# Victarry/Image-Generation-models

Measured on AMD Instinct MI355X. Metric: ddpm_cifar10_32x32_train_images_per_sec, higher is better.
Workload: dtype bf16; 1 GPU; DDPM CIFAR-10 32x32, UNet 128/1-2-4, T=1000 (BASELINE configs[1]): train step B=128/GPU + hipGraph denoise step B=64; per_gpu_batch=128, global_batch=128, parallelism=dp1, step_launch=hipGraph replay, denoise_batch=64, rccl_ranks=1, state_finite=True, matmul=bf16 MFMA, fp32 accumulate

## Files before the change

### image-generation-models_amd/csrc/small_channel.hip

```cpp
#include <stdlib.h>
#include "common.h"

namespace {

typedef float f32x4 __attribute__((ext_vector_type(4)));

template <bool B16> __device__ __forceinline__ f32x4 ldq(const void* base, size_t off) {
    if constexpr (B16) {
        const uint2 u = *reinterpret_cast<const uint2*>(reinterpret_cast<const uint16_t*>(base) + off);
        return f32x4{__uint_as_float(u.x << 16), __uint_as_float(u.x & 0xffff0000u), __uint_as_float(u.y << 16), __uint_as_float(u.y & 0xffff0000u)};
    } else return *reinterpret_cast<const f32x4*>(reinterpret_cast<const float*>(base) + off);
}
template <bool B16> __device__ __forceinline__ void stq(void* base, size_t off, const f32x4& v) {
    if constexpr (B16) *reinterpret_cast<uint2*>(reinterpret_cast<uint16_t*>(base) + off) = make_uint2(pack_bf16(v.x, v.y), pack_bf16(v.z, v.w));
    else *reinterpret_cast<f32x4*>(reinterpret_cast<float*>(base) + off) = v;
}

constexpr int WG_BLOCKS = 768;

template <bool POW2>
__device__ __forceinline__ void decode_px(int m, int H, int W, int w_sh, int hw_sh, int& n, int& yy, int& xx) {
    if constexpr (POW2) {
        n = m >> hw_sh; const int rem = m & ((1 << hw_sh) - 1);
        yy = rem >> w_sh; xx = rem & ((1 << w_sh) - 1);
    } else {
        n = m / (H * W); const int rem = m - n * (H * W);
        yy = rem / W; xx = rem - yy * W;
    }
}

template <int CIN, bool VEC>
__device__ __forceinline__ f32x4 load_small(const float* __restrict__ x, int ldx, int n, int iy, int ix, int H, int W) {
    const bool ok = iy >= 0 && iy < H && ix >= 0 && ix < W;
    const float* p = x + (size_t)((n * H + (ok ? iy : 0)) * W + (ok ? ix : 0)) * ldx;
    f32x4 v = {0.f, 0.f, 0.f, 0.f};
    if constexpr (VEC) v = *reinterpret_cast<const f32x4*>(p);
    else { v.x = p[0]; if (CIN > 1) v.y = p[1]; if (CIN > 2) v.z = p[2]; if (CIN > 3) v.w = p[3]; }
    const float k = ok ? 1.f : 0.f;
    return v * k;
}

template <int CIN, int KS, bool POW2, bool VEC>
__global__ __launch_bounds__(256) void small_cin_fwd_kernel(int N, int H, int W, int Cout, const float* __restrict__ x, int ldx,
                                                            const float* __restrict__ w, const float* __restrict__ bias,
                                                            float* __restrict__ y, int ldy, int w_sh, int hw_sh) {
    constexpr int NT = KS * KS;
    const int nq = Cout / 4;
    const int q = threadIdx.x % nq, psub = threadIdx.x / nq, pp = 256 / nq;
    f32x4 wr[NT * CIN];
#pragma unroll
    for (int i = 0; i < NT * CIN; ++i) wr[i] = *reinterpret_cast<const f32x4*>(w + (size_t)i * Cout + 4 * q);
// ... 112 lines not shown
#pragma unroll
            for (int k = 0; k < 3; ++k) a[i] += *reinterpret_cast<const f32x4*>(&red[((k * NA + i) * nq + l) * 4]);
    }
}

template <int CIN, int KS, bool POW2, bool VEC>
__global__ __launch_bounds__(256) void small_cin_wgrad_kernel(int N, int H, int W, int Cout, const float* __restrict__ x, int ldx,
                                                              const float* __restrict__ dy, int lddy, float* __restrict__ dW,
                                                              float* __restrict__ ws, int w_sh, int hw_sh) {
    constexpr int NT = KS * KS, NA = NT * CIN;
    extern __shared__ float red[];
    const int nq = Cout / 4;
    const int q = threadIdx.x % nq, psub = threadIdx.x / nq, pp = 256 / nq;
    f32x4 acc[NA];
#pragma unroll
    for (int i = 0; i < NA; ++i) acc[i] = f32x4{0.f, 0.f, 0.f, 0.f};
    const int M = N * H * W;
    const int per = (M + gridDim.x - 1) / gridDim.x;
    const int mb = blockIdx.x * per, me = min(M, mb + per);
    int m = mb + psub;
    f32x4 g = *reinterpret_cast<const f32x4*>(dy + (size_t)min(m, M - 1) * lddy + 4 * q);
    for (; m < me; m += pp) {
        const f32x4 gnext = *reinterpret_cast<const f32x4*>(dy + (size_t)min(m + pp, M - 1) * lddy + 4 * q);
        int n, yy, xx;
        decode_px<POW2>(m, H, W, w_sh, hw_sh, n, yy, xx);
#pragma unroll
        for (int tp = 0; tp < NT; ++tp) {
            const f32x4 xv = load_small<CIN, VEC>(x, ldx, n, yy + tp / KS - KS / 2, xx + tp % KS - KS / 2, H, W);
#pragma unroll
            for (int ci = 0; ci < CIN; ++ci) acc[tp * CIN + ci] += xv[ci] * g;
        }
        g = gnext;
    }
    block_reduce_quads<NA>(acc, nq, red);
    if (threadIdx.x < nq) {
        if (ws) {
            float* out = ws + (size_t)blockIdx.x * NA * Cout;
#pragma unroll
            for (int i = 0; i < NA; ++i) *reinterpret_cast<f32x4*>(out + (size_t)i * Cout + 4 * q) = acc[i];
        } else {
#pragma unroll
            for (int i = 0; i < NA; ++i)
#pragma unroll
                for (int k = 0; k < 4; ++k) atomicAdd(dW + (size_t)i * Cout + 4 * q + k, acc[i][k]);
        }
    }
}

template <int CIN, bool DY16 = false>
__global__ __launch_bounds__(256) void small_cin3x3_wgrad_tiled_kernel(int N, int H, int W, int Cout, const float* __restrict__ x, int ldx,
                                                                       const void* __restrict__ dy, int lddy, float* __restrict__ dW,
                                                                       float* __restrict__ ws, int w_sh, int ntiles) {
    constexpr int NA = 9 * CIN;
    extern __shared__ __attribute__((aligned(16))) float smem[];
    const int nq = Cout / 4;
    const int q = threadIdx.x % nq, psub = threadIdx.x / nq, pp = 256 / nq;
    const int rows = 64 >> w_sh, W2 = W + 2, HP = (rows + 2) * W2, tiles_per_img = H / rows;
    float* red = smem;
    float* halo_s = smem + (size_t)3 * NA * nq * 4;
    f32x4 acc[NA];
#pragma unroll
    for (int i = 0; i < NA; ++i) acc[i] = f32x4{0.f, 0.f, 0.f, 0.f};
    const int hp = threadIdx.x, hy = hp / W2, hx = hp - hy * W2;
    auto fetch = [&](int tile) -> f32x4 {
        const int n = tile / tiles_per_img, y0 = (tile - n * tiles_per_img) * rows;
        const int iy = y0 + hy - 1, ix = hx - 1;
// ... 22 lines not shown
#pragma unroll
            for (int k = 0; k < MAXPX; ++k) {
                const int px = base + k * pp;
                if (px < 64) {
                    const int ty = px >> w_sh, tx = px & (W - 1);
#pragma unroll
                    for (int tp = 0; tp < 9; ++tp) {
                        const f32x4 xv = *reinterpret_cast<const f32x4*>(hs + (size_t)((ty + tp / 3) * W2 + tx + tp % 3) * 4);
#pragma unroll
                        for (int ci = 0; ci < CIN; ++ci) acc[tp * CIN + ci] += xv[ci] * g[k];
                    }
                }
            }
        }
        buf ^= 1;
        if (hp < HP) *reinterpret_cast<f32x4*>(halo_s + ((size_t)buf * HP + hp) * 4) = nxt;
        __syncthreads();
    }
    block_reduce_quads<NA>(acc, nq, red);
    if (threadIdx.x < nq) {
        if (ws) {
            float* out = ws + (size_t)blockIdx.x * NA * Cout;
#pragma unroll
            for (int i = 0; i < NA; ++i) *reinterpret_cast<f32x4*>(out + (size_t)i * Cout + 4 * q) = acc[i];
        } else {
#pragma unroll
            for (int i = 0; i < NA; ++i)
#pragma unroll
                for (int k = 0; k < 4; ++k) atomicAdd(dW + (size_t)i * Cout + 4 * q + k, acc[i][k]);
        }
    }
}

__global__ __launch_bounds__(256) void partial_sum_kernel(const float* __restrict__ ws, int nparts, int nout, float* __restrict__ out, int rows4) {
    __shared__ float red[8][32];
    const int ol = threadIdx.x & 31, grp = threadIdx.x >> 5;
    const int o = blockIdx.x * 32 + ol;
    float s = 0.f;
    if (o < nout) {
        float s0 = 0.f, s1 = 0.f, s2 = 0.f, s3 = 0.f;
        int p = grp;
        for (; p + 56 < nparts; p += 64) {
            float v[8];
#pragma unroll
            for (int u = 0; u < 8; ++u) v[u] = ws[(size_t)(p + 8 * u) * nout + o];
            s0 += v[0] + v[4]; s1 += v[1] + v[5]; s2 += v[2] + v[6]; s3 += v[3] + v[7];
        }
        for (; p < nparts; p += 8) s0 += ws[(size_t)p * nout + o];
        s = (s0 + s1) + (s2 + s3);
    }
    red[grp][ol] = s;
    __syncthreads();
    if (grp == 0 && o < nout) {
#pragma unroll
        for (int g = 1; g < 8; ++g) s += red[g][ol];
        if (rows4 > 0) { if ((o & 3) < rows4) out[(o >> 2) * rows4 + (o & 3)] += s; }
        else out[o] += s;
    }
}

template <int CK, bool X16 = false>
__global__ __launch_bounds__(256) void small_cout_fwd_kernel(int M, int Cs, const void* __restrict__ x, int ldx,
                                                             const float* __restrict__ w, const float* __restrict__ bias,
                                                             float* __restrict__ y, int ldy) {
    const int sub = threadIdx.x & 7, pl = threadIdx.x >> 3;
    f32x4 wr[CK][4];
// ... 167 lines not shown
    const int mb = blockIdx.x * per, me = min(M, mb + per);
    int m = mb + psub;
    f32x4 xv = ldq<X16>(x, (size_t)min(m, M - 1) * ldx + 4 * q);
    for (; m < me; m += pp) {
        const f32x4 xnext = ldq<X16>(x, (size_t)min(m + pp, M - 1) * ldx + 4 * q);
        const float* gp = dy + (size_t)m * lddy;
        const f32x4 g = {gp[0], Cs > 1 ? gp[1] : 0.f, Cs > 2 ? gp[2] : 0.f, Cs > 3 ? gp[3] : 0.f};
#pragma unroll
        for (int e = 0; e < 4; ++e) acc[e] += xv[e] * g;
        if constexpr (DG) {
            f32x4 o;
#pragma unroll
            for (int e = 0; e < 4; ++e) { const f32x4 pr = g * wr[e]; o[e] = (pr.x + pr.y) + (pr.z + pr.w); }
            const size_t po = (size_t)m * lddx + 4 * q;
            if (dacc) o += ldq<DX16>(dx, po);
            stq<DX16>(dx, po, o);
        }
        xv = xnext;
    }
    block_reduce_quads<4>(acc, nq, red);
    if (threadIdx.x < nq) {
        if (ws) {
            float* out = ws + (size_t)blockIdx.x * C * 4;
#pragma unroll
            for (int e = 0; e < 4; ++e) *reinterpret_cast<f32x4*>(out + (size_t)(4 * q + e) * 4) = acc[e];
        } else {
#pragma unroll
            for (int e = 0; e < 4; ++e)
                for (int j = 0; j < Cs; ++j) atomicAdd(dW + (size_t)(4 * q + e) * Cs + j, acc[e][j]);
        }
    }
}

int log2_exact(int v) { int s = 0; while ((1 << s) < v) ++s; return (1 << s) == v ? s : -1; }

}

extern "C" size_t mi_conv_small_wgrad_workspace(int outputs) { return (size_t)WG_BLOCKS * (size_t)outputs * sizeof(float); }

namespace {
bool cin_tiled_geom(int ks, int H, int W, int ldx, const void* x) {
    const int w_sh = log2_exact(W), hw_sh = log2_exact(H * W);
    const int rows = w_sh >= 0 && W <= 64 ? 64 / W : 0;
    return ks == 3 && w_sh >= 0 && hw_sh >= 0 && ldx == 4 && ((uintptr_t)x & 15) == 0 && rows >= 1 && H % rows == 0 && (rows + 2) * (W + 2) <= 256;
}
}

extern "C" int mi_conv_small_cin_bf16_supported(int ks, int N, int H, int W, int Cin, int Cout, int ldx) {
    static const int tiled = (int)mi_knob("MI_SMALL_CIN_TILED", 1);
    return (tiled && N > 0 && Cin >= 1 && Cin <= 4 && (Cout == 64 || Cout == 128 || Cout == 256) && ((long)N * H * W) % 64 == 0 && cin_tiled_geom(ks, H, W, ldx, nullptr) &&
            (size_t)3 * 9 * Cin * (Cout / 4) * 16 <= 48 * 1024) ? 1 : 0;
}

extern "C" int mi_conv_small_cin_fwd_io(int ks, int N, int H, int W, int Cin, int Cout, const float* x, int ldx, const float* w,
                                        const float* bias, void* yv, int ldy, int y_bf16, void* stream) {
    MI_REQUIRE(x && w && yv && (ks == 1 || ks == 3) && Cin >= 1 && Cin <= 4 && Cout >= 4 && Cout % 4 == 0 && Cout <= 1024 && 256 % (Cout / 4) == 0 &&
               ldy % 4 == 0 && (((uintptr_t)yv & (y_bf16 ? 7 : 15)) | ((uintptr_t)w & 15)) == 0,
               "needs ks 1|3, Cin <= 4, Cout a multiple of 4 with Cout/4 dividing 256, 16-byte aligned y / w");
    float* y = (float*)yv;
    const int pp = 256 / (Cout / 4);
    long blocks = ((long)N * H * W + 2 * pp - 1) / (2 * pp); if (blocks > 4096) blocks = 4096;
    const int w_sh = log2_exact(W), hw_sh = log2_exact(H * W);
    const bool pow2 = w_sh >= 0 && hw_sh >= 0;
    const bool vec = ldx % 4 == 0 && ((uintptr_t)x & 15) == 0;
    hipStream_t st = (hipStream_t)stream;
    {
        static const int tiled = (int)mi_knob("MI_SMALL_CIN_TILED", 1);
        const int rows = w_sh >= 0 && W <= 64 ? 64 / W : 0;
// ... 55 lines not shown
    hipStream_t st = (hipStream_t)stream;
#define MI_TILED2(CIN) do { \
        if (y3_bf16) hipLaunchKernelGGL((small_cin3x3_fwd_tiled_kernel<CIN, true, true>), dim3(grid), dim3(256), lds, st, N, H, W, Cout, x, ldx, w3, bias3, y3, ldy3, w_sh, ntiles, w1, bias1, y1, ldy1, (unsigned long long*)ch.zero, (int)(ch.zero_bytes / 8), ch.gsrc, ch.gidx, ch.gdst, ch.grow, ch.gB); \
        else hipLaunchKernelGGL((small_cin3x3_fwd_tiled_kernel<CIN, false, true>), dim3(grid), dim3(256), lds, st, N, H, W, Cout, x, ldx, w3, bias3, y3, ldy3, w_sh, ntiles, w1, bias1, y1, ldy1, (unsigned long long*)ch.zero, (int)(ch.zero_bytes / 8), ch.gsrc, ch.gidx, ch.gdst, ch.grow, ch.gB); } while (0)
    switch (Cin) { case 1: MI_TILED2(1); break; case 2: MI_TILED2(2); break; case 3: MI_TILED2(3); break; default: MI_TILED2(4); break; }
#undef MI_TILED2
    MI_LAUNCH_CHECK();
    return 0;
}
extern "C" int mi_conv_small_cin_fwd(int ks, int N, int H, int W, int Cin, int Cout, const float* x, int ldx, const float* w,
                                     const float* bias, float* y, int ldy, void* stream) {
    return mi_conv_small_cin_fwd_io(ks, N, H, W, Cin, Cout, x, ldx, w, bias, y, ldy, 0, stream);
}

extern "C" int mi_conv_small_cin_wgrad_io(int ks, int N, int H, int W, int Cin, int Cout, const float* x, int ldx, const void* dyv,
                                          int lddy, int dy_bf16, float* dW, void* workspace, size_t ws_bytes, void* stream) {
    const int na = ks * ks * Cin;
    MI_REQUIRE(x && dyv && dW && (ks == 1 || ks == 3) && Cin >= 1 && Cin <= 4 && (Cout == 64 || Cout == 128 || Cout == 256) && lddy % 4 == 0 &&
               ((uintptr_t)dyv & (dy_bf16 ? 7 : 15)) == 0 && (size_t)3 * na * (Cout / 4) * 16 <= 48 * 1024,
               "needs ks 1|3, Cin <= 4, Cout in {64, 128, 256} with 3 ks ks Cin (Cout / 4) float4 of reduce area <= 48 KiB (3x3: Cin Cout <= 455), 16-byte aligned dy rows");
    const float* dy = (const float*)dyv;
    float* ws = (workspace && ws_bytes >= mi_conv_small_wgrad_workspace(na * Cout)) ? (float*)workspace : nullptr;
    const int w_sh = log2_exact(W), hw_sh = log2_exact(H * W);
    const bool pow2 = w_sh >= 0 && hw_sh >= 0;
    const bool vec = ldx % 4 == 0 && ((uintptr_t)x & 15) == 0;
    const size_t lds = (size_t)3 * na * (Cout / 4) * 4 * sizeof(float);
    hipStream_t st = (hipStream_t)stream;
    {
        static const int tiled = (int)mi_knob("MI_SMALL_CIN_TILED", 1);
        const int rows = w_sh >= 0 && W <= 64 ? 64 / W : 0;
        if (tiled && cin_tiled_geom(ks, H, W, ldx, x) && (Cout >= 128 || dy_bf16) && ((long)N * H * W) % 64 == 0) {
            const int ntiles = N * H * W / 64;
            const size_t lds2 = lds + (size_t)2 * (rows + 2) * (W + 2) * 16;
#define MI_TILED(CIN) do { \
                if (dy_bf16) hipLaunchKernelGGL((small_cin3x3_wgrad_tiled_kernel<CIN, true>), dim3(WG_BLOCKS), dim3(256), lds2, st, N, H, W, Cout, x, ldx, dyv, lddy, dW, ws, w_sh, ntiles); \
                else hipLaunchKernelGGL((small_cin3x3_wgrad_tiled_kernel<CIN, false>), dim3(WG_BLOCKS), dim3(256), lds2, st, N, H, W, Cout, x, ldx, dyv, lddy, dW, ws, w_sh, ntiles); } while (0)
            switch (Cin) { case 1: MI_TILED(1); break; case 2: MI_TILED(2); break; case 3: MI_TILED(3); break; default: MI_TILED(4); break; }
#undef MI_TILED
            if (ws) hipLaunchKernelGGL(partial_sum_kernel, dim3((na * Cout + 31) / 32), dim3(256), 0, st, ws, WG_BLOCKS, na * Cout, dW, 0);
            MI_LAUNCH_CHECK();
            return 0;
        }
    }
    MI_REQUIRE(!dy_bf16, "bf16 dy: only on the whole-row-tile kernel (mi_conv_small_cin_bf16_supported)");
#define MI_GO(CIN, KS) do { \
        if (pow2 && vec) hipLaunchKernelGGL((small_cin_wgrad_kernel<CIN, KS, true, true>), dim3(WG_BLOCKS), dim3(256), lds, st, N, H, W, Cout, x, ldx, dy, lddy, dW, ws, w_sh, hw_sh); \
        else if (vec) hipLaunchKernelGGL((small_cin_wgrad_kernel<CIN, KS, false, true>), dim3(WG_BLOCKS), dim3(256), lds, st, N, H, W, Cout, x, ldx, dy, lddy, dW, ws, 0, 0); \
        else hipLaunchKernelGGL((small_cin_wgrad_kernel<CIN, KS, false, false>), dim3(WG_BLOCKS), dim3(256), lds, st, N, H, W, Cout, x, ldx, dy, lddy, dW, ws, 0, 0); } while (0)
    if (ks == 3) MI_GO_CIN(3); else MI_GO_CIN(1);
#undef MI_GO
#undef MI_GO_CIN
    if (ws) hipLaunchKernelGGL(partial_sum_kernel, dim3((na * Cout + 31) / 32), dim3(256), 0, st, ws, WG_BLOCKS, na * Cout, dW, 0);
    MI_LAUNCH_CHECK();
    return 0;
}
extern "C" int mi_conv_small_cin_wgrad(int ks, int N, int H, int W, int Cin, int Cout, const float* x, int ldx, const float* dy,
                                       int lddy, float* dW, void* workspace, size_t ws_bytes, void* stream) {
    return mi_conv_small_cin_wgrad_io(ks, N, H, W, Cin, Cout, x, ldx, dy, lddy, 0, dW, workspace, ws_bytes, stream);
}

extern "C" int mi_conv3x3_small_cin_fwd(int N, int H, int W, int Cin, int Cout, const float* x, int ldx, const float* w,
                                        const float* bias, float* y, int ldy, void* stream) {
    return mi_conv_small_cin_fwd(3, N, H, W, Cin, Cout, x, ldx, w, bias, y, ldy, stream);
}
extern "C" int mi_conv3x3_small_cin_wgrad(int N, int H, int W, int Cin, int Cout, const float* x, int ldx, const float* dy,
                                          int lddy, float* dW, void* stream) {
    return mi_conv_small_cin_wgrad(3, N, H, W, Cin, Cout, x, ldx, dy, lddy, dW, nullptr, 0, stream);
}

extern "C" int mi_conv1x1_small_cout_io(int op, int M, int C, int Cs, const void* a, int lda, const float* b, int ldb,
                                        const float* w, const float* bias, void* out, int ldo, int accumulate, int wide_bf16,
                                        void* workspace, size_t ws_bytes, void* stream) {
    MI_REQUIRE(a && out && (op == 2 || w) && Cs >= 1 && Cs <= 4 && (C == 32 || C == 64 || C == 128 || C == 256) && M > 0,
               "needs Cs <= 4 and C in {32, 64, 128, 256}");
    hipStream_t st = (hipStream_t)stream;
    const uintptr_t wal = wide_bf16 ? 7 : 15;
    if (op == 0) {
        MI_REQUIRE(C <= 128 && lda % 4 == 0 && ((uintptr_t)a & wal) == 0, "forward: C <= 128, 16-byte (bf16: 8-byte) aligned x rows");
        int blocks = (M + 31) / 32; if (blocks > 1024) blocks = 1024;
#define MI_FWD(CK) do { \
            if (wide_bf16) hipLaunchKernelGGL((small_cout_fwd_kernel<CK, true>), dim3(blocks), dim3(256), 0, st, M, Cs, a, lda, w, bias, (float*)out, ldo); \
            else hipLaunchKernelGGL((small_cout_fwd_kernel<CK, false>), dim3(blocks), dim3(256), 0, st, M, Cs, a, lda, w, bias, (float*)out, ldo); } while (0)
        if (C == 128) MI_FWD(4); else if (C == 64) MI_FWD(2); else MI_FWD(1);
#undef MI_FWD
    } else if (op == 1) {
        MI_REQUIRE(ldo % 4 == 0 && ((uintptr_t)out & wal) == 0, "dgrad: 16-byte (bf16: 8-byte) aligned dx rows");
        const int pp = 256 / (C / 4);
        long blocks = ((long)M + pp - 1) / pp; if (blocks > 4096) blocks = 4096;
        if (wide_bf16) hipLaunchKernelGGL(small_cout_dgrad_kernel<true>, dim3((unsigned)blocks), dim3(256), 0, st, M, C, Cs, (const float*)a, lda, w, out, ldo, accumulate);
        else hipLaunchKernelGGL(small_cout_dgrad_kernel<false>, dim3((unsigned)blocks), dim3(256), 0, st, M, C, Cs, (const float*)a, lda, w, out, ldo, accumulate);
    } else if (op == 2) {
        MI_REQUIRE(b && C >= 64 && lda % 4 == 0 && ((uintptr_t)a & wal) == 0, "wgrad: needs dy, C in {64, 128, 256}, aligned x rows");
        float* ws = (workspace && ws_bytes >= mi_conv_small_wgrad_workspace(C * 4)) ? (float*)workspace : nullptr;
        const size_t lds = (size_t)3 * 4 * (C / 4) * 4 * sizeof(float);
        if (wide_bf16) hipLaunchKernelGGL(small_cout_wgrad_kernel<true>, dim3(WG_BLOCKS), dim3(256), lds, st, M, C, Cs, a, lda, b, ldb, (float*)out, ws);
        else hipLaunchKernelGGL(small_cout_wgrad_kernel<false>, dim3(WG_BLOCKS), dim3(256), lds, st, M, C, Cs, a, lda, b, ldb, (float*)out, ws);
        if (ws) hipLaunchKernelGGL(partial_sum_kernel, dim3((C * 4 + 31) / 32), dim3(256), 0, st, ws, WG_BLOCKS, C * 4, (float*)out, Cs);
    } else {
        return mi_set_error(-1, "mi_conv1x1_small_cout: op must be 0, 1 or 2");
    }
    MI_LAUNCH_CHECK();
    return 0;
}

extern "C" int mi_conv1x1_small_cout_gn_supported(int C, int Cs, int G) {
    return ((C == 64 || C == 128) && Cs >= 1 && Cs <= 4 && G > 0 && C % G == 0 && (C / G) % 16 == 0) ? 1 : 0;
}
extern "C" int mi_conv1x1_small_cout_gn_fwd(int M, int HW, int C, int Cs, const void* x_bf16, int ldx, const void* sums, const float* gamma,
                                            const float* beta, int G, float eps, const float* w, const float* bias, float* y, int ldy, void* stream) {
    MI_REQUIRE(x_bf16 && sums && gamma && beta && w && y && M > 0 && HW > 0 && M % HW == 0 && mi_conv1x1_small_cout_gn_supported(C, Cs, G) &&
               ldx % 4 == 0 && ldy == 4 && (((uintptr_t)x_bf16 & 7) | ((uintptr_t)sums & 15) | ((uintptr_t)gamma & 15) | ((uintptr_t)beta & 15) | ((uintptr_t)y & 15)) == 0,
               "needs C in {64, 128}, (C / G) % 16 == 0, Cs <= 4, y as padded 4-channel pixels, aligned operands");
    int ppw = 32;
    while ((long)M / ppw > 768 && HW % (2 * ppw) == 0) ppw *= 2;
    const int blocks = (M + ppw - 1) / ppw;
    hipStream_t st = (hipStream_t)stream;
    if (C == 128) hipLaunchKernelGGL((small_cout_fwd_gn_kernel<4>), dim3(blocks), dim3(256), 0, st, M, HW, Cs, (const uint16_t*)x_bf16, ldx, (const long long*)sums, gamma, beta, G, eps, w, bias, y, ldy, ppw);
    else hipLaunchKernelGGL((small_cout_fwd_gn_kernel<2>), dim3(blocks), dim3(256), 0, st, M, HW, Cs, (const uint16_t*)x_bf16, ldx, (const long long*)sums, gamma, beta, G, eps, w, bias, y, ldy, ppw);
    MI_LAUNCH_CHECK();
    return 0;
}

extern "C" int mi_conv1x1_small_cout_bwd(int M, int C, int Cs, const void* x, int ldx, int x_bf16, const float* dy, int lddy, const float* w,
                                         float* dW, void* dx, int lddx, int dx_bf16, int accumulate_dx, void* workspace, size_t ws_bytes, void* stream) {
    MI_REQUIRE(x && dy && w && dW && dx && Cs >= 1 && Cs <= 4 && (C == 64 || C == 128 || C == 256) && M > 0 && ldx % 4 == 0 && lddx % 4 == 0 &&
               ((uintptr_t)x & (x_bf16 ? 7 : 15)) == 0 && ((uintptr_t)dx & (dx_bf16 ? 7 : 15)) == 0, "needs Cs <= 4, C in {64, 128, 256}, aligned rows");
    hipStream_t st = (hipStream_t)stream;
    float* ws = (workspace && ws_bytes >= mi_conv_small_wgrad_workspace(C * 4)) ? (float*)workspace : nullptr;
    const size_t lds = (size_t)3 * 4 * (C / 4) * 4 * sizeof(float);
#define MI_BWD(X16, D16) hipLaunchKernelGGL((small_cout_wgrad_kernel<X16, true, D16>), dim3(WG_BLOCKS), dim3(256), lds, st, M, C, Cs, x, ldx, dy, lddy, dW, ws, w, dx, lddx, accumulate_dx)
    if (x_bf16) { if (dx_bf16) MI_BWD(true, true); else MI_BWD(true, false); }
    else { if (dx_bf16) MI_BWD(false, true); else MI_BWD(false, false); }
#undef MI_BWD
    if (ws) hipLaunchKernelGGL(partial_sum_kernel, dim3((C * 4 + 31) / 32), dim3(256), 0, st, ws, WG_BLOCKS, C * 4, dW, Cs);
    MI_LAUNCH_CHECK();
    return 0;
}

extern "C" int mi_conv1x1_small_cout_ws(int op, int M, int C, int Cs, const float* a, int lda, const float* b, int ldb,
                                        const float* w, const float* bias, float* out, int ldo, int accumulate,
                                        void* workspace, size_t ws_bytes, void* stream) {
    return mi_conv1x1_small_cout_io(op, M, C, Cs, a, lda, b, ldb, w, bias, out, ldo, accumulate, 0, workspace, ws_bytes, stream);
}

extern "C" int mi_conv1x1_small_cout(int op, int M, int C, int Cs, const float* a, int lda, const float* b, int ldb,
                                     const float* w, const float* bias, float* out, int ldo, int accumulate, void* stream) {
    return mi_conv1x1_small_cout_ws(op, M, C, Cs, a, lda, b, ldb, w, bias, out, ldo, accumulate, nullptr, 0, stream);
}
```

### image-generation-models_amd/src/ops/lib.py

```python
from __future__ import annotations

import ctypes as C
import os

_PKG_ROOT = os.path.dirname(os.path.dirname(os.path.dirname(os.path.abspath(__file__))))
_LIB = None


def library_path() -> str:
    return os.environ.get("MI_DDPM_LIB", os.path.join(_PKG_ROOT, "lib", "libmi_ddpm.so"))


class MiConvDesc(C.Structure):
    _fields_ = [(n, C.c_int) for n in (
        "N", "IH", "IW", "OH", "OW", "K", "Nc", "KH", "KW", "stride", "pad", "transposed", "w_kn", "mode",
        "K1", "ldx", "ldx2", "ldy", "ldr", "accumulate")]


class MiWgradDesc(C.Structure):
    _fields_ = [(n, C.c_int) for n in (
        "N", "GH", "GW", "DH", "DW", "Ci", "Cj", "KH", "KW", "stride", "pad", "gather_i", "mode", "I1",
        "ldp", "ldp2", "ldq")]


# ... 143 lines not shown
    "mi_conv_small_cin_bf16_supported": [_I, _I, _I, _I, _I, _I, _I],
    "mi_conv_small_cin_fwd": [_I, _I, _I, _I, _I, _I, _P, _I, _P, _P, _P, _I, _P],
    "mi_conv_small_cin_wgrad": [_I, _I, _I, _I, _I, _I, _P, _I, _P, _I, _P, _P, _Z, _P],
    "mi_conv_wgrad": [C.POINTER(MiWgradDesc), _P, _P, _P, _P, _P],
    "mi_conv3x3_wgrad": [C.POINTER(MiWgradDesc), _P, _P, _P, _P, _P],
    "mi_conv3x3_wgrad_supported": [C.POINTER(MiWgradDesc)],
    "mi_conv3x3_wgrad_ws": [C.POINTER(MiWgradDesc), _P, _P, _P, _P, _P, _Z, _P],
    "mi_conv3x3_wgrad_bias": [C.POINTER(MiWgradDesc), _P, _P, _P, _P, _P, _P, _Z, _P],
    "mi_colsum": [_I, _I, _P, _I, _P, _P],
    "mi_colsum_ordered": [_I, _I, _P, _I, _P, _P, _Z, _P],
    "mi_conv_wgrad_slabs": [C.POINTER(MiWgradDesc), _P, _P, _P, _P, _P, _Z, _P],
    "mi_gn_mish_fwd": [C.POINTER(MiGnDesc), _P, _P, _P, _P, _I, _P, _P, _P, _P],
    "mi_gn_mish_bwd": [C.POINTER(MiGnDesc), _P, _P, _P, _P, _P, _I, _P, _I, _P, _P, _P, _I, _P, _P],
    "mi_chan_layernorm_fwd": [_I, _I, _P, _I, _P, _P, _F, _P, _I, _P],
    "mi_chan_layernorm_bwd": [_I, _I, _P, _I, _P, _F, _P, _I, _P, _I, _I, _P, _P, _P],
    "mi_linattn_fwd": [_I, _I, _I, _P, _P, _P, _P, _P],
    "mi_linattn_bwd": [_I, _I, _I, _P, _P, _P, _P, _P, _P],
    "mi_vq_partials": [_I],
    "mi_vq_nearest_fwd": [_I, _I, _I, _P, _I, _P, _P, _P, _I, _P, _P],
    "mi_vq_bwd": [_I, _I, _I, _P, _I, _P, _P, _F, _F, _P, _P, _I, _I, _P, _P],
    "mi_vq_scatter_rows": [_I, _I, _I, _P, _I, _P, _P, _P],
    "mi_small_gemm": [_I, _I, _I, _I, _I, _P, _I, _P, _I, _P, _P, _I, _I, _I, _P],
    "mi_small_gemm_supported": [_I, _I, _I, _I, _I, _I, _I],
    "mi_linattn_fwd_io": [_I, _I, _I, _P, _P, _P, _P, _I, _P],
    "mi_linattn_bwd_io": [_I, _I, _I, _P, _P, _P, _P, _P, _I, _P],
    "mi_linattn_fwd_ws": [_I, _I, _I, _P, _P, _P, _P, _I, _P, _Z, _P],
    "mi_linattn_bwd_ws": [_I, _I, _I, _P, _P, _P, _P, _P, _I, _P, _Z, _P],
    "mi_chan_layernorm_fwd_io": [_I, _I, _P, _I, _P, _P, _F, _P, _I, _I, _P],
    "mi_chan_layernorm_bwd_io": [_I, _I, _P, _I, _P, _F, _P, _I, _P, _I, _I, _P, _P, _I, _P],
    "mi_chan_layernorm_bwd_part": [_I, _I, _P, _I, _P, _F, _P, _I, _P, _I, _I, _P, _I, _P],
    "mi_chan_layernorm_bwd_out": [_I, _I, _P, _I, _P, _F, _P, _I, _P, _I, _P, _I, _P, _P, _P, _I, _P],
    "mi_chan_layernorm_bwd_pipelined": [_I, _P, _P, _P, _P, _I, _I, _I, _I, _I],
    "mi_debug_ln_bwd_pipeline": [_I],
    "mi_rowsum_batch": [_I, _P, _P],
    "mi_f32_to_bf16_colsum_part": [_Z, _I, _P, _I, _P, _I, _P, _Z, C.POINTER(C.c_int), _P],
    "mi_time_embed": [_I, _I, _P, _P, _P],
    "mi_sample_norm_supported": [_I, _I, _I],
    "mi_sample_norm_fwd": [_I, _I, _I, _P, _P, _P, _P, _P, _F, _P],
    "mi_sample_norm_bwd": [_I, _I, _I, _P, _P, _P, _P, _P, _P, _P, _P, _P],
    "mi_sample_norm_bwd2": [_I, _I, _I, _P, _P, _P, _P, _P, _P, _P, _P, _P],
    "mi_leaky_relu_fwd": [_Z, _P, _P, _F, _P],
    "mi_leaky_relu_bwd": [_Z, _P, _P, _P, _F, _P],
    "mi_tanh_fwd": [_Z, _P, _P, _P],
    "mi_tanh_bwd": [_Z, _P, _P, _P, _P],
    "mi_lerp_rows": [_I, _Z, _P, _P, _P, _P, _P],
    "mi_gp_penalty": [_I, _Z, _P, _P, _P, _F, _P, _P],
    "mi_batchnorm_workspace": [_I],
    "mi_batchnorm_fwd": [_I, _I, _P, _P, _P, _P, _P, _P, _P, _P, _F, _F, _I, _P, _P],
    "mi_batchnorm_bwd": [_I, _I, _P, _P, _P, _P, _P, _P, _P, _P, _P, _P],
    "mi_vae_latent_fwd": [_I, _I, _P, _I, _P, _P, _P, _P],
    "mi_vae_latent_bwd": [_I, _I, _P, _I, _P, _P, _F, _P, _P, _I, _P],
    "mi_cvae_pack_input": [_I, _I, _I, _I, _P, _P, _P, _I, _P],
    "mi_cvae_latent_fwd": [_I, _I, _I, _P, _I, _P, _P, _P, _P, _P, _P],
    "mi_cvae_latent_bwd": [_I, _I, _I, _P, _I, _P, _P, _P, _I, _F, _P, _P, _P, _P],
    "mi_latent_disc_supported": [_I, _I, _I],
    "mi_latent_disc_fwd": [_I, _I, _I, _P, _I, _P, _I, _P, _P, _P, _I, _F, _F, _P, _P, _P, _P, _P, _P],
    "mi_latent_disc_bwd": [_I, _I, _I, _P, _I, _P, _I, _P, _P, _P, _I, _F, _P, _P, _P, _F, _I, _P, _I, _F, _I, _P],
    "mi_latent_disc_ln_supported": [_I, _I, _I, _I],
    "mi_latent_disc_ln_fwd": [_I, _I, _I, _I, _P, _I, _P, _I, _P, _I, _F, _F, _P, _P, _P],
    "mi_latent_disc_ln_bwd": [_I, _I, _I, _I, _P, _I, _P, _I, _P, _I, _F, _F, _F, _F, _P, _P, _P, _F, _I, _P, _I, _F, _I, _P],
    "mi_bn_seg_rows_per_workgroup": [_I, _I],
    "mi_bn_seg_fwd": [_I, _I, _I, _P, _P, _P, _P, _P, _P, _P, _P, _F, _F, _I, _I, _F, _P, _P],
    "mi_bn_seg_bwd": [_I, _I, _I, _P, _P, _P, _P, _P, _P, _P, _P, _P, _I, _I, _F, _P, _P],
    "mi_adv_loss": [_I, _I, _I, C.POINTER(C.c_int), _F, _P, _I, _P, _P, _P, _I, _P],
    "mi_info_latent": [_I, _I, _I, _I, _I, _P, _P, _I, _P, _I, _P, _I, _P],
    "mi_info_head_supported": [_I, _I, _I, _I, _I, _I, _I],
# ... 121 lines not shown
```

### include/mi_ddpm.h

```cpp
#ifndef MI_DDPM_H
#define MI_DDPM_H
#include <stddef.h>
#include <stdint.h>

#ifdef __cplusplus
extern "C" {
#endif

#define MI_ABI_VERSION 4
#define MI_MODE_FP32 0
#define MI_MODE_BF16 1

int mi_abi_version(void);
const char* mi_last_error(void);

typedef struct MiConvDesc {
    int N;
    int IH, IW;
    int OH, OW;
    int K;
    int Nc;
    int KH, KW, stride, pad;
    int transposed;
    int w_kn;
// ... 249 lines not shown
int mi_gn_mish_fwd_io(const MiGnDesc* d, const void* x, const float* gamma, const float* beta, const float* temb,
                      int ldt, const float* residual, void* y, float* stats, int io, void* stream);
int mi_gn_mish_fwd_dual(const MiGnDesc* d, const void* x, const float* gamma, const float* beta,
                        const float* temb, int ldt, const float* residual, void* y, void* y16, int ldy16,
                        float* stats, int io, void* stream);
int mi_gn_mish_apply_sums(const MiGnDesc* d, const void* x, const void* sums, const float* gamma, const float* beta, const float* temb,
                          int ldt, const float* residual, void* y, int y_is_bf16, void* y_bf16, int ldy16, float* stats, void* stream);
int mi_gn_stats_coef(const MiGnDesc* d, const void* x, const float* gamma, const float* beta, const float* temb, int ldt,
                     float* stats, float* coef, int x_is_bf16, void* stream);
int mi_gn_mish_bwd_io(const MiGnDesc* d, const void* x, const float* stats, const float* gamma, const float* beta,
                      const void* dout, int lddo, void* dx, int lddx, float* dgamma, float* dbeta, float* dtemb,
                      int ldt, float* dbias, int io, void* stream);

int mi_chan_layernorm_fwd(int M, int C, const float* x, int ldx, const float* g, const float* b,
                          float eps, float* y, int ldy, void* stream);
int mi_chan_layernorm_bwd(int M, int C, const float* x, int ldx, const float* g, float eps,
                          const float* dy, int lddy, float* dx, int lddx, int accumulate_dx,
                          float* dg, float* db, void* stream);
int mi_chan_layernorm_fwd_io(int M, int C, const float* x, int ldx, const float* g, const float* b,
                             float eps, void* y, int ldy, int y16, void* stream);
int mi_chan_layernorm_bwd_io(int M, int C, const float* x, int ldx, const float* g, float eps,
                             const void* dy, int lddy, float* dx, int lddx, int accumulate_dx,
                             float* dg, float* db, int dy16, void* stream);
int mi_chan_layernorm_bwd_part_rows(int M, int C);
int mi_chan_layernorm_bwd_part(int M, int C, const float* x, int ldx, const float* g, float eps,
                               const void* dy, int lddy, float* dx, int lddx, int accumulate_dx,
                               float* part, int dy16, void* stream);
int mi_chan_layernorm_bwd_out(int M, int C, const float* x, int ldx, const float* g, float eps,
                              const void* dy, int lddy, const float* dx_in, int lddx_in, float* dx_out, int lddx_out,
                              float* dg, float* db, float* part, int dy16, void* stream);
int mi_chan_layernorm_bwd_pipelined(int C, const void* x, const void* dy, const void* dx, const void* dx_in, int ldx, int lddy,
                                    int lddx, int lddx_in, int dy16);
int mi_debug_ln_bwd_pipeline(int on);

int mi_linattn_fwd(int B, int n, int heads, const float* qkv, float* out, float* ctx,
                   float* kstat, void* stream);
int mi_linattn_bwd(int B, int n, int heads, const float* qkv, const float* ctx,
                   const float* kstat, const float* dout, float* dqkv, void* stream);
int mi_linattn_fwd_io(int B, int n, int heads, const void* qkv, void* out, float* ctx, float* kstat, int b16,
                      void* stream);
int mi_linattn_bwd_io(int B, int n, int heads, const void* qkv, const float* ctx, const float* kstat,
                      const void* dout, void* dqkv, int b16, void* stream);
size_t mi_linattn_workspace(int B, int n, int heads);
int mi_linattn_fwd_ws(int B, int n, int heads, const void* qkv, void* out, float* ctx, float* kstat, int b16,
                      void* workspace, size_t ws_bytes, void* stream);
int mi_linattn_bwd_ws(int B, int n, int heads, const void* qkv, const float* ctx, const float* kstat,
                      const void* dout, void* dqkv, int b16, void* workspace, size_t ws_bytes, void* stream);

int mi_small_gemm(int ta, int tb, int I, int J, int K, const float* A, int lda, const float* B, int ldb,
                  const float* bias, float* C, int ldc, int accumulate, int allow_split, void* stream);
int mi_small_gemm_supported(int ta, int tb, int I, int J, int K, int lda, int ldb);

int mi_vq_partials(int M);
int mi_vq_nearest_fwd(int M, int D, int K, const float* z, int ldz, const float* codebook, int* idx, float* zq, int ldq,
                      float* loss_partial, void* stream);
int mi_vq_bwd(int M, int D, int K, const float* z, int ldz, const float* codebook, const int* idx, float g_vq, float g_commit,
              const float* g_dev, float* dz, int lddz, int accumulate_dz, float* dcodebook, void* stream);
int mi_vq_scatter_rows(int M, int D, int K, const float* src, int ld, const int* idx, float* table, void* stream);

int mi_sample_norm_supported(int N, int P, int C);
int mi_sample_norm_fwd(int N, int P, int C, const float* x, const float* gamma, const float* beta, float* y, float* stats, float eps,
                       void* stream);
int mi_sample_norm_bwd(int N, int P, int C, const float* x, const float* stats, const float* gamma, const float* dy, const float* extra_dx,
                       float* dx, float* dgamma, float* dbeta, void* stream);
int mi_sample_norm_bwd2(int N, int P, int C, const float* x, const float* stats, const float* gamma, const float* dy, const float* u,
                        float* adj_dy, float* adj_x, float* dgamma, void* stream);
// ... 191 lines not shown
```

Before: 27990 images/s.

## Add load-ahead software-pipelined variants of small-channel wgrad kernels

Adds new small-Cin and small-Cout weight-gradient kernels that keep several rows of dy/x loads in flight (U-deep register rings) before consuming them. A tiled 3x3 variant also prefetches the next tile's dy rows ahead of the halo compute. These are enabled by default through a debug toggle. The goal is to hide global memory latency in these bandwidth-bound reductions, at the cost of more registers and possible occupancy loss. The Cin=3 fp32 path instantiates the CIN=2 template.

```diff
diff --git a/image-generation-models_amd/csrc/small_channel.hip b/image-generation-models_amd/csrc/small_channel.hip
--- a/image-generation-models_amd/csrc/small_channel.hip
+++ b/image-generation-models_amd/csrc/small_channel.hip
@@ -1,4 +1,5 @@
 #include <stdlib.h>
+#include <type_traits>
 #include "common.h"
 
 namespace {
@@ -17,6 +18,8 @@
 }
 
 constexpr int WG_BLOCKS = 768;
+constexpr int COUT_WG_U = 8, COUT_WG_U_ACC = 4, CIN_WG_U = 4;
+constexpr int WGT_NPRE16 = 4, WGT_NPRE32 = 4;
 
 template <bool POW2>
 __device__ __forceinline__ void decode_px(int m, int H, int W, int w_sh, int hw_sh, int& n, int& yy, int& xx) {
@@ -195,6 +198,57 @@
         }
         g = gnext;
     }
+    block_reduce_quads<NA>(acc, nq, red);
+    if (threadIdx.x < nq) {
+        if (ws) {
+            float* out = ws + (size_t)blockIdx.x * NA * Cout;
+#pragma unroll
+            for (int i = 0; i < NA; ++i) *reinterpret_cast<f32x4*>(out + (size_t)i * Cout + 4 * q) = acc[i];
+        } else {
+#pragma unroll
+            for (int i = 0; i < NA; ++i)
+#pragma unroll
+                for (int k = 0; k < 4; ++k) atomicAdd(dW + (size_t)i * Cout + 4 * q + k, acc[i][k]);
+        }
+    }
+}
+
+template <int CIN, bool VEC, int U>
+__global__ __launch_bounds__(256) void small_cin_wgrad_ahead_kernel(int M, int Cout, const float* __restrict__ x, int ldx,
+                                                                    const float* __restrict__ dy, int lddy, float* __restrict__ dW,
+                                                                    float* __restrict__ ws) {
+    constexpr int NA = CIN;
+    extern __shared__ float red[];
+    const int nq = Cout / 4;
+    const int q = threadIdx.x % nq, psub = threadIdx.x / nq, pp = 256 / nq;
+    f32x4 acc[NA];
+#pragma unroll
+    for (int i = 0; i < NA; ++i) acc[i] = f32x4{0.f, 0.f, 0.f, 0.f};
+    const int per = (M + gridDim.x - 1) / gridDim.x;
+    const int mb = blockIdx.x * per, me = min(M, mb + per);
+    int m = mb + psub;
+    f32x4 gr[U], xr[U];
+    auto request = [&](int s, int mm) {
+        const size_t r = (size_t)min(mm, M - 1);
+        gr[s] = *reinterpret_cast<const f32x4*>(dy + r * lddy + 4 * q);
+        const float* p = x + r * ldx;
+        if constexpr (VEC) xr[s] = *reinterpret_cast<const f32x4*>(p);
+        else xr[s] = f32x4{p[0], CIN > 1 ? p[1] : 0.f, CIN > 2 ? p[2] : 0.f, CIN > 3 ? p[3] : 0.f};
+    };
+    auto consume = [&](int s) {
+        const f32x4 g = gr[s], xv = xr[s];
+#pragma unroll
+        for (int ci = 0; ci < CIN; ++ci) acc[ci] += xv[ci] * g;
+    };
+#pragma unroll
+    for (int s = 0; s < U; ++s) request(s, m + s * pp);
+    while (m + (U - 1) * pp < me) {
+#pragma unroll
+        for (int s = 0; s < U; ++s) { consume(s); request(s, m + (s + U) * pp); }
+        m += U * pp;
+    }
+#pragma unroll
+    for (int s = 0; s < U - 1; ++s) if (m + s * pp < me) consume(s);
     block_reduce_quads<NA>(acc, nq, red);
     if (threadIdx.x < nq) {
         if (ws) {
@@ -283,6 +337,97 @@
     }
 }
 
+template <int CIN, bool DY16, int NPRE>
+__global__ __launch_bounds__(256) void small_cin3x3_wgrad_tiled_ahead_kernel(int N, int H, int W, int Cout, const float* __restrict__ x, int ldx,
+                                                                             const void* __restrict__ dy, int lddy, float* __restrict__ dW,
+                                                                             float* __restrict__ ws, int w_sh, int ntiles) {
+    constexpr int NA = 9 * CIN, NPX = 8;
+    typedef std::conditional_t<DY16, uint2, f32x4> raw_t;
+    extern __shared__ __attribute__((aligned(16))) float smem[];
+    const int nq = 32;
+    const int q = threadIdx.x & 31, psub = threadIdx.x >> 5;
+    const int rows = 64 >> w_sh, W2 = W + 2, HP = (rows + 2) * W2, tiles_per_img = H / rows;
+    float* red = smem;
+    float* halo_s = smem + (size_t)3 * NA * nq * 4;
+    f32x4 acc[NA];
+#pragma unroll
+    for (int i = 0; i < NA; ++i) acc[i] = f32x4{0.f, 0.f, 0.f, 0.f};
+    const int hp = threadIdx.x, hy = hp / W2, hx = hp - hy * W2;
+    auto fetch = [&](int tile) -> f32x4 {
+        const int n = tile / tiles_per_img, y0 = (tile - n * tiles_per_img) * rows;
+        const int iy = y0 + hy - 1, ix = hx - 1;
+        const bool ok = hp < HP && tile < ntiles && iy >= 0 && iy < H && ix >= 0 && ix < W;
+        const f32x4 v = *reinterpret_cast<const f32x4*>(x + (size_t)((n * H + (ok ? iy : 0)) * W + (ok ? ix : 0)) * (ok ? ldx : 0));
+        return v * (ok ? 1.f : 0.f);
+    };
+    auto row = [&](int tile, int k) -> raw_t {
+        const size_t off = ((size_t)tile * 64 + psub + k * 8) * lddy + 4 * q;
+        if constexpr (DY16) return *reinterpret_cast<const uint2*>(reinterpret_cast<const uint16_t*>(dy) + off);
+        else return *reinterpret_cast<const f32x4*>(reinterpret_cast<const float*>(dy) + off);
+    };
+    auto widen = [](const raw_t& r) -> f32x4 {
+        if constexpr (DY16) return f32x4{__uint_as_float(r.x << 16), __uint_as_float(r.x & 0xffff0000u), __uint_as_float(r.y << 16), __uint_as_float(r.y & 0xffff0000u)};
+        else return r;
+    };
+    const int per = (ntiles + gridDim.x - 1) / gridDim.x;
+    const int tb = blockIdx.x * per, te = min(ntiles, tb + per);
+    int buf = 0;
+    f32x4 nxt = fetch(tb < te ? tb : ntiles);
+    raw_t g[NPX], gn[NPRE];
+    {
+        const int t0 = tb < te ? tb : 0;
+#pragma unroll
+        for (int k = 0; k < NPRE; ++k) gn[k] = row(t0, k);
+    }
+    if (hp < HP) *reinterpret_cast<f32x4*>(halo_s + (size_t)hp * 4) = nxt;
+    __syncthreads();
+    for (int tile = tb; tile < te; ++tile) {
+        nxt = fetch(tile + 1 < te ? tile + 1 : ntiles);
+#pragma unroll
+        for (int k = 0; k < NPRE; ++k) g[k] = gn[k];
+#pragma unroll
+        for (int k = NPRE; k < NPX; ++k) g[k] = row(tile, k);
+        {
+            const int t1 = tile + 1 < te ? tile + 1 : tile;
+#pragma unroll
+            for (int k = 0; k < NPRE; ++k) gn[k] = row(t1, k);
+        }
+        const float* hs = halo_s + (size_t)buf * HP * 4;
+        int lim = 64, p0 = psub;
+        asm volatile("" : "+s"(lim), "+v"(p0));
+#pragma unroll
+        for (int k = 0; k < NPX; ++k) {
+            const int px = p0 + k * 8;
+            if (px < lim) {
+                const int ty = px >> w_sh, tx = px & (W - 1);
+                const f32x4 gk = widen(g[k]);
+#pragma unroll
+                for (int tp = 0; tp < 9; ++tp) {
+                    const f32x4 xv = *reinterpret_cast<const f32x4*>(hs + (size_t)((ty + tp / 3) * W2 + tx + tp % 3) * 4);
+#pragma unroll
+                    for (int ci = 0; ci < CIN; ++ci) acc[tp * CIN + ci] += xv[ci] * gk;
+                }
+            }
+        }
+        buf ^= 1;
+        if (hp < HP) *reinterpret_cast<f32x4*>(halo_s + ((size_t)buf * HP + hp) * 4) = nxt;
+        __syncthreads();
+    }
+    block_reduce_quads<NA>(acc, nq, red);
+    if (threadIdx.x < nq) {
+        if (ws) {
+            float* out = ws + (size_t)blockIdx.x * NA * Cout;
+#pragma unroll
+            for (int i = 0; i < NA; ++i) *reinterpret_cast<f32x4*>(out + (size_t)i * Cout + 4 * q) = acc[i];
+        } else {
+#pragma unroll
+            for (int i = 0; i < NA; ++i)
+#pragma unroll
+                for (int k = 0; k < 4; ++k) atomicAdd(dW + (size_t)i * Cout + 4 * q + k, acc[i][k]);
+        }
+    }
+}
+
 __global__ __launch_bounds__(256) void partial_sum_kernel(const float* __restrict__ ws, int nparts, int nout, float* __restrict__ out, int rows4) {
     __shared__ float red[8][32];
     const int ol = threadIdx.x & 31, grp = threadIdx.x >> 5;
@@ -516,8 +661,83 @@
     }
 }
 
+template <bool X16, bool DG, bool DX16, bool DACC, bool GV, int U>
+__global__ __launch_bounds__(256) void small_cout_wgrad_ahead_kernel(int M, int C, int Cs, const void* __restrict__ x, int ldx,
+                                                                     const float* __restrict__ dy, int lddy, float* __restrict__ dW,
+                                                                     float* __restrict__ ws, const float* __restrict__ w = nullptr,
+                                                                     void* __restrict__ dx = nullptr, int lddx = 0) {
+    extern __shared__ float red[];
+    const int nq = C / 4;
+    const int q = threadIdx.x % nq, psub = threadIdx.x / nq, pp = 256 / nq;
+    f32x4 acc[4];
+#pragma unroll
+    for (int e = 0; e < 4; ++e) acc[e] = f32x4{0.f, 0.f, 0.f, 0.f};
+    const int per = (M + gridDim.x - 1) / gridDim.x;
+    const int mb = blockIdx.x * per, me = min(M, mb + per);
+    int m = mb + psub;
+    const int j1 = min(1, Cs - 1), j2 = min(2, Cs - 1), j3 = min(3, Cs - 1);
+    f32x4 xr[U], gr[U], dr[DACC ? U : 1];
+    auto request = [&](int s, int mm) {
+        const size_t r = (size_t)min(mm, M - 1);
+        xr[s] = ldq<X16>(x, r * ldx + 4 * q);
+        const float* gp = dy + r * lddy;
+        if constexpr (GV) gr[s] = *reinterpret_cast<const f32x4*>(gp);
+        else gr[s] = f32x4{gp[0], gp[j1], gp[j2], gp[j3]};
+        if constexpr (DACC) dr[s] = ldq<DX16>(dx, r * lddx + 4 * q);
+    };
+#pragma unroll
+    for (int s = 0; s < U; ++s) request(s, m + s * pp);
+    f32x4 wr[DG ? 4 : 1];
+    if constexpr (DG) {
+#pragma unroll
+        for (int e = 0; e < 4; ++e) {
+            const float* wp = w + (size_t)(4 * q + e) * Cs;
+            wr[e] = f32x4{wp[0], Cs > 1 ? wp[1] : 0.f, Cs > 2 ? wp[2] : 0.f, Cs > 3 ? wp[3] : 0.f};
+        }
+    }
+    auto consume = [&](int s, int mm) {
+        const f32x4 xv = xr[s], gw = gr[s];
+        const f32x4 g = {gw.x, Cs > 1 ? gw.y : 0.f, Cs > 2 ? gw.z : 0.f, Cs > 3 ? gw.w : 0.f};
+#pragma unroll
+        for (int e = 0; e < 4; ++e) acc[e] += xv[e] * g;
+        if constexpr (DG) {
+            f32x4 o;
+#pragma unroll
+            for (int e = 0; e < 4; ++e) { const f32x4 pr = g * wr[e]; o[e] = (pr.x + pr.y) + (pr.z + pr.w); }
+            if constexpr (DACC) o += dr[s];
+            stq<DX16>(dx, (size_t)mm * lddx + 4 * q, o);
+        }
+    };
+    while (m + (U - 1) * pp < me) {
+#pragma unroll
+        for (int s = 0; s < U; ++s) { consume(s, m + s * pp); request(s, m + (s + U) * pp); }
+        m += U * pp;
+    }
+#pragma unroll
+    for (int s = 0; s < U - 1; ++s) if (m + s * pp < me) consume(s, m + s * pp);
+    block_reduce_quads<4>(acc, nq, red);
+    if (threadIdx.x < nq) {
+        if (ws) {
+            float* out = ws + (size_t)blockIdx.x * C * 4;
+#pragma unroll
+            for (int e = 0; e < 4; ++e) *reinterpret_cast<f32x4*>(out + (size_t)(4 * q + e) * 4) = acc[e];
+        } else {
+#pragma unroll
+            for (int e = 0; e < 4; ++e)
+                for (int j = 0; j < Cs; ++j) atomicAdd(dW + (size_t)(4 * q + e) * Cs + j, acc[e][j]);
+        }
+    }
+}
+
 int log2_exact(int v) { int s = 0; while ((1 << s) < v) ++s; return (1 << s) == v ? s : -1; }
 
+}
+
+static int g_mi_stream_ahead = 1;
+extern "C" int mi_debug_stream_ahead(int on) {
+    const int was = g_mi_stream_ahead;
+    g_mi_stream_ahead = on != 0;
+    return was;
 }
 
 extern "C" size_t mi_conv_small_wgrad_workspace(int outputs) { return (size_t)WG_BLOCKS * (size_t)outputs * sizeof(float); }
@@ -639,6 +859,16 @@
         if (tiled && cin_tiled_geom(ks, H, W, ldx, x) && (Cout >= 128 || dy_bf16) && ((long)N * H * W) % 64 == 0) {
             const int ntiles = N * H * W / 64;
             const size_t lds2 = lds + (size_t)2 * (rows + 2) * (W + 2) * 16;
+            if (g_mi_stream_ahead && Cout == 128 && ntiles > 0 && (dy_bf16 || Cin <= 2)) {
+#define MI_TILED_AHEAD(CIN) do { \
+                if (dy_bf16) hipLaunchKernelGGL((small_cin3x3_wgrad_tiled_ahead_kernel<CIN, true, WGT_NPRE16>), dim3(WG_BLOCKS), dim3(256), lds2, st, N, H, W, Cout, x, ldx, dyv, lddy, dW, ws, w_sh, ntiles); \
+                else hipLaunchKernelGGL((small_cin3x3_wgrad_tiled_ahead_kernel<(CIN < 3 ? CIN : 2), false, WGT_NPRE32>), dim3(WG_BLOCKS), dim3(256), lds2, st, N, H, W, Cout, x, ldx, dyv, lddy, dW, ws, w_sh, ntiles); } while (0)
+                switch (Cin) { case 1: MI_TILED_AHEAD(1); break; case 2: MI_TILED_AHEAD(2); break; default: MI_TILED_AHEAD(3); break; }
+#undef MI_TILED_AHEAD
+                if (ws) hipLaunchKernelGGL(partial_sum_kernel, dim3((na * Cout + 31) / 32), dim3(256), 0, st, ws, WG_BLOCKS, na * Cout, dW, 0);
+                MI_LAUNCH_CHECK();
+                return 0;
+            }
 #define MI_TILED(CIN) do { \
                 if (dy_bf16) hipLaunchKernelGGL((small_cin3x3_wgrad_tiled_kernel<CIN, true>), dim3(WG_BLOCKS), dim3(256), lds2, st, N, H, W, Cout, x, ldx, dyv, lddy, dW, ws, w_sh, ntiles); \
                 else hipLaunchKernelGGL((small_cin3x3_wgrad_tiled_kernel<CIN, false>), dim3(WG_BLOCKS), dim3(256), lds2, st, N, H, W, Cout, x, ldx, dyv, lddy, dW, ws, w_sh, ntiles); } while (0)
@@ -654,9 +884,15 @@
         if (pow2 && vec) hipLaunchKernelGGL((small_cin_wgrad_kernel<CIN, KS, true, true>), dim3(WG_BLOCKS), dim3(256), lds, st, N, H, W, Cout, x, ldx, dy, lddy, dW, ws, w_sh, hw_sh); \
         else if (vec) hipLaunchKernelGGL((small_cin_wgrad_kernel<CIN, KS, false, true>), dim3(WG_BLOCKS), dim3(256), lds, st, N, H, W, Cout, x, ldx, dy, lddy, dW, ws, 0, 0); \
         else hipLaunchKernelGGL((small_cin_wgrad_kernel<CIN, KS, false, false>), dim3(WG_BLOCKS), dim3(256), lds, st, N, H, W, Cout, x, ldx, dy, lddy, dW, ws, 0, 0); } while (0)
-    if (ks == 3) MI_GO_CIN(3); else MI_GO_CIN(1);
+#define MI_GO_AHEAD(CIN) do { \
+        if (vec) hipLaunchKernelGGL((small_cin_wgrad_ahead_kernel<CIN, true, CIN_WG_U>), dim3(WG_BLOCKS), dim3(256), lds, st, N * H * W, Cout, x, ldx, dy, lddy, dW, ws); \
+        else hipLaunchKernelGGL((small_cin_wgrad_ahead_kernel<CIN, false, CIN_WG_U>), dim3(WG_BLOCKS), dim3(256), lds, st, N * H * W, Cout, x, ldx, dy, lddy, dW, ws); } while (0)
+    if (ks == 3) MI_GO_CIN(3);
+    else if (!g_mi_stream_ahead || N * H * W < 1) MI_GO_CIN(1);
+    else switch (Cin) { case 1: MI_GO_AHEAD(1); break; case 2: MI_GO_AHEAD(2); break; case 3: MI_GO_AHEAD(3); break; default: MI_GO_AHEAD(4); break; }
 #undef MI_GO
 #undef MI_GO_CIN
+#undef MI_GO_AHEAD
     if (ws) hipLaunchKernelGGL(partial_sum_kernel, dim3((na * Cout + 31) / 32), dim3(256), 0, st, ws, WG_BLOCKS, na * Cout, dW, 0);
     MI_LAUNCH_CHECK();
     return 0;
@@ -700,7 +936,14 @@
         MI_REQUIRE(b && C >= 64 && lda % 4 == 0 && ((uintptr_t)a & wal) == 0, "wgrad: needs dy, C in {64, 128, 256}, aligned x rows");
         float* ws = (workspace && ws_bytes >= mi_conv_small_wgrad_workspace(C * 4)) ? (float*)workspace : nullptr;
         const size_t lds = (size_t)3 * 4 * (C / 4) * 4 * sizeof(float);
-        if (wide_bf16) hipLaunchKernelGGL(small_cout_wgrad_kernel<true>, dim3(WG_BLOCKS), dim3(256), lds, st, M, C, Cs, a, lda, b, ldb, (float*)out, ws);
+        if (g_mi_stream_ahead) {
+            const bool gv = ldb == 4 && ((uintptr_t)b & 15) == 0;
+#define MI_WG_AHEAD(X16, GV) hipLaunchKernelGGL((small_cout_wgrad_ahead_kernel<X16, false, false, false, GV, COUT_WG_U>), dim3(WG_BLOCKS), dim3(256), lds, st, M, C, Cs, a, lda, b, ldb, (float*)out, ws)
+            if (wide_bf16) { if (gv) MI_WG_AHEAD(true, true); else MI_WG_AHEAD(true, false); }
+            else { if (gv) MI_WG_AHEAD(false, true); else MI_WG_AHEAD(false, false); }
+#undef MI_WG_AHEAD
+        }
+        else if (wide_bf16) hipLaunchKernelGGL(small_cout_wgrad_kernel<true>, dim3(WG_BLOCKS), dim3(256), lds, st, M, C, Cs, a, lda, b, ldb, (float*)out, ws);
         else hipLaunchKernelGGL(small_cout_wgrad_kernel<false>, dim3(WG_BLOCKS), dim3(256), lds, st, M, C, Cs, a, lda, b, ldb, (float*)out, ws);
         if (ws) hipLaunchKernelGGL(partial_sum_kernel, dim3((C * 4 + 31) / 32), dim3(256), 0, st, ws, WG_BLOCKS, C * 4, (float*)out, Cs);
     } else {
@@ -736,9 +979,20 @@
     float* ws = (workspace && ws_bytes >= mi_conv_small_wgrad_workspace(C * 4)) ? (float*)workspace : nullptr;
     const size_t lds = (size_t)3 * 4 * (C / 4) * 4 * sizeof(float);
 #define MI_BWD(X16, D16) hipLaunchKernelGGL((small_cout_wgrad_kernel<X16, true, D16>), dim3(WG_BLOCKS), dim3(256), lds, st, M, C, Cs, x, ldx, dy, lddy, dW, ws, w, dx, lddx, accumulate_dx)
-    if (x_bf16) { if (dx_bf16) MI_BWD(true, true); else MI_BWD(true, false); }
+#define MI_BWD_AHEAD(X16, D16, DACC, GV) hipLaunchKernelGGL((small_cout_wgrad_ahead_kernel<X16, true, D16, DACC, GV, (DACC ? COUT_WG_U_ACC : COUT_WG_U)>), dim3(WG_BLOCKS), dim3(256), lds, st, M, C, Cs, x, ldx, dy, lddy, dW, ws, w, dx, lddx)
+#define MI_BWD_AHEAD2(X16, D16) do { \
+        if (accumulate_dx) { if (gv) MI_BWD_AHEAD(X16, D16, true, true); else MI_BWD_AHEAD(X16, D16, true, false); } \
+        else { if (gv) MI_BWD_AHEAD(X16, D16, false, true); else MI_BWD_AHEAD(X16, D16, false, false); } } while (0)
+    if (g_mi_stream_ahead) {
+        const bool gv = lddy == 4 && ((uintptr_t)dy & 15) == 0;
+        if (x_bf16) { if (dx_bf16) MI_BWD_AHEAD2(true, true); else MI_BWD_AHEAD2(true, false); }
+        else { if (dx_bf16) MI_BWD_AHEAD2(false, true); else MI_BWD_AHEAD2(false, false); }
+    }
+    else if (x_bf16) { if (dx_bf16) MI_BWD(true, true); else MI_BWD(true, false); }
     else { if (dx_bf16) MI_BWD(false, true); else MI_BWD(false, false); }
 #undef MI_BWD
+#undef MI_BWD_AHEAD
+#undef MI_BWD_AHEAD2
     if (ws) hipLaunchKernelGGL(partial_sum_kernel, dim3((C * 4 + 31) / 32), dim3(256), 0, st, ws, WG_BLOCKS, C * 4, dW, Cs);
     MI_LAUNCH_CHECK();
     return 0;
diff --git a/image-generation-models_amd/src/ops/lib.py b/image-generation-models_amd/src/ops/lib.py
--- a/image-generation-models_amd/src/ops/lib.py
+++ b/image-generation-models_amd/src/ops/lib.py
@@ -199,6 +199,7 @@
     "mi_chan_layernorm_bwd_out": [_I, _I, _P, _I, _P, _F, _P, _I, _P, _I, _P, _I, _P, _P, _P, _I, _P],
     "mi_chan_layernorm_bwd_pipelined": [_I, _P, _P, _P, _P, _I, _I, _I, _I, _I],
     "mi_debug_ln_bwd_pipeline": [_I],
+    "mi_debug_stream_ahead": [_I],
     "mi_rowsum_batch": [_I, _P, _P],
     "mi_f32_to_bf16_colsum_part": [_Z, _I, _P, _I, _P, _I, _P, _Z, C.POINTER(C.c_int), _P],
     "mi_time_embed": [_I, _I, _P, _P, _P],
diff --git a/include/mi_ddpm.h b/include/mi_ddpm.h
--- a/include/mi_ddpm.h
+++ b/include/mi_ddpm.h
@@ -305,6 +305,7 @@
 int mi_chan_layernorm_bwd_pipelined(int C, const void* x, const void* dy, const void* dx, const void* dx_in, int ldx, int lddy,
                                     int lddx, int lddx_in, int dy16);
 int mi_debug_ln_bwd_pipeline(int on);
+int mi_debug_stream_ahead(int on);
 
 int mi_linattn_fwd(int B, int n, int heads, const float* qkv, float* out, float* ctx,
                    float* kstat, void* stream);
```

Result: no change. 27990 images/s (median of 3 runs) (+0.0%).
